# TIERS/multi-modal-loam

Hardware: AMD Instinct MI355X
Metric: scans/s (feature-extract+kNN+10 GN iters) on 16-ring x1800 + Livox 24k fused cloud (higher is better)
Workload: dtype f32/f64; 1 GPU; BASELINE configs[1]: fused VLP-16 16x1800 + Livox Horizon 24000 scan (52800 pts), local map 200000 pts, 1 association pass (thres_dist 25), 10 GN iterations, W=1; resident_slots=8192, stream_lanes=2, distinct_scans=64, map_tiles_touched=43, map_tiles_complete=43, parallelism=scan-sharded x1, device=AMD Radeon Graphics, cus=256

## Files before the change

multi-modal-loam_amd/csrc/lidar_eval.h:

```cpp
#pragma once
#include <math.h>
#include <stddef.h>

#include "mml_internal.h"

namespace {

#ifndef MML_SOLVE_THREADS
#define MML_SOLVE_THREADS 128
#endif
constexpr int SOLVE_THREADS = MML_SOLVE_THREADS;
constexpr int SOLVE_WAVES = SOLVE_THREADS / 64;
constexpr int MAXW = 8;
constexpr double kLidarM = 1.5e-3;

struct Pose {
    double R[9];
    double t[3];
    double tb[3];
    double Jl[9];
};

__device__ void quat_to_R(double qx, double qy, double qz, double qw, double* R) {
    const double tx = 2 * qx, ty = 2 * qy, tz = 2 * qz;
// ... 113 lines not shown
        Pw[0] = __builtin_fma(P.R[2], cz, __builtin_fma(P.R[1], cy, __builtin_fma(P.R[0], cx, P.t[0])));
        Pw[1] = __builtin_fma(P.R[5], cz, __builtin_fma(P.R[4], cy, __builtin_fma(P.R[3], cx, P.t[1])));
        Pw[2] = __builtin_fma(P.R[8], cz, __builtin_fma(P.R[7], cy, __builtin_fma(P.R[6], cx, P.t[2])));
        double l12, il12, a012, ia012, s12, is12, rs, sm14;
        const double dx = ax - bx, dy = ay - by, dz = az - bz;
        sqrt_pair(__builtin_fma(dz, dz, __builtin_fma(dy, dy, dx * dx)), l12, il12);
        const double pax = Pw[0] - ax, pay = Pw[1] - ay, paz = Pw[2] - az, pbx = Pw[0] - bx, pby = Pw[1] - by, pbz = Pw[2] - bz;
        const double c0 = __builtin_fma(pax, pby, -(pbx * pay));
        const double c1 = __builtin_fma(pax, pbz, -(pbx * paz));
        const double c2 = __builtin_fma(pay, pbz, -(pby * paz));
        sqrt_pair(__builtin_fma(c2, c2, __builtin_fma(c1, c1, c0 * c0)), a012, ia012);
        const double ld2 = a012 * il12;
        const double s = __builtin_fma(Pw[2], Pw[2], __builtin_fma(Pw[1], Pw[1], Pw[0] * Pw[0]));
        sqrt_pair(s, s12, is12);
        sqrt_pair(s12, rs, sm14);
        const double weight = 1.0 - 0.9 * fabs(ld2) * sm14;
        const double r = ka * weight * ld2;
        const double ux = c2 * ia012, uy = -c1 * ia012, uz = c0 * ia012;
        double gl[3] = {__builtin_fma(dy, uz, -(dz * uy)) * il12, __builtin_fma(dz, ux, -(dx * uz)) * il12, __builtin_fma(dx, uy, -(dy * ux)) * il12};
        const double sm54 = sm14 * (is12 * is12);
        double gr[3];
        for (int c = 0; c < 3; ++c) {
            double gw = (-0.9) * __builtin_fma(fabs(ld2) * (-0.5) * sm54, Pw[c], sm14 * gl[c]);
            gr[c] = ka * __builtin_fma(ld2, gw, weight * gl[c]);
        }
        double J[6];
        row_jacobian(P, Pw, gr, J);
        double rho0, rho1;
        huber(r * r, huber_delta, rho0, rho1);
        acc[27] += 0.5 * rho0;
        accum(acc, J, r, rho1);
    }
    const double kb = w_tan / kLidarM;
    MmlPlaneFactor nxt;
    if ((int)threadIdx.x < npf) nxt = pf[threadIdx.x];
    for (int i = threadIdx.x; i < npf; i += SOLVE_THREADS) {
        const MmlPlaneFactor f = nxt;
        if (i + SOLVE_THREADS < npf) nxt = pf[i + SOLVE_THREADS];
        if (f.src < 0 || !(fabs(f.error) > 1e-5)) continue;
        const double cx = f.ori[0], cy = f.ori[1], cz = f.ori[2];
        double Pw[3];
        Pw[0] = __builtin_fma(P.R[2], cz, __builtin_fma(P.R[1], cy, __builtin_fma(P.R[0], cx, P.t[0])));
        Pw[1] = __builtin_fma(P.R[5], cz, __builtin_fma(P.R[4], cy, __builtin_fma(P.R[3], cx, P.t[1])));
        Pw[2] = __builtin_fma(P.R[8], cz, __builtin_fma(P.R[7], cy, __builtin_fma(P.R[6], cx, P.t[2])));
        const double d[3] = {Pw[0] - f.proj[0], Pw[1] - f.proj[1], Pw[2] - f.proj[2]};
        double nd, ind, s12, is12, rs, sm14;
        sqrt_pair(__builtin_fma(d[2], d[2], __builtin_fma(d[1], d[1], d[0] * d[0])), nd, ind);
        const double s = __builtin_fma(Pw[2], Pw[2], __builtin_fma(Pw[1], Pw[1], Pw[0] * Pw[0]));
        sqrt_pair(s, s12, is12);
        sqrt_pair(s12, rs, sm14);
        const double weight = 1.0 - 0.9 * nd * sm14;
        const double sm54 = sm14 * (is12 * is12);
        double gw[3];
        const double gwa = sm14 * ind, gwb = nd * (-0.5) * sm54;
        for (int c = 0; c < 3; ++c) gw[c] = (-0.9) * __builtin_fma(gwb, Pw[c], gwa * d[c]);
        const double w[3] = {f.omega[0], f.omega[1], f.omega[2]};
        double rows[3][3];
        int nrows = 1;
        rows[0][0] = ka * w[0];
        rows[0][1] = ka * w[1];
        rows[0][2] = ka * w[2];
        if (kb != 0.0) {
            double h[3] = {0, 0, 0};
            if (fabs(w[0]) <= fabs(w[1]) && fabs(w[0]) <= fabs(w[2]))
                h[0] = 1;
            else if (fabs(w[1]) <= fabs(w[2]))
                h[1] = 1;
            else
                h[2] = 1;
            double t0 = w[1] * h[2] - w[2] * h[1], t1 = w[2] * h[0] - w[0] * h[2], t2 = w[0] * h[1] - w[1] * h[0];
            double n, in;
            sqrt_pair((t0 * t0 + t1 * t1) + t2 * t2, n, in);
            t0 *= in;
            t1 *= in;
            t2 *= in;
            rows[1][0] = kb * t0;
            rows[1][1] = kb * t1;
            rows[1][2] = kb * t2;
            rows[2][0] = kb * (w[1] * t2 - w[2] * t1);
            rows[2][1] = kb * (w[2] * t0 - w[0] * t2);
            rows[2][2] = kb * (w[0] * t1 - w[1] * t0);
            nrows = 3;
        }
        double rr[3], sq = 0;
        for (int q = 0; q < nrows; ++q) {
            rr[q] = weight * __builtin_fma(rows[q][2], d[2], __builtin_fma(rows[q][1], d[1], rows[q][0] * d[0]));
            sq = __builtin_fma(rr[q], rr[q], sq);
        }
        double rho0, rho1;
        huber(sq, huber_delta, rho0, rho1);
        acc[27] += 0.5 * rho0;
        for (int q = 0; q < nrows; ++q) {
            const double rd = __builtin_fma(rows[q][2], d[2], __builtin_fma(rows[q][1], d[1], rows[q][0] * d[0]));
            double gr[3] = {__builtin_fma(rd, gw[0], weight * rows[q][0]), __builtin_fma(rd, gw[1], weight * rows[q][1]),
                            __builtin_fma(rd, gw[2], weight * rows[q][2])};
            double J[6];
            row_jacobian(P, Pw, gr, J);
            accum(acc, J, rr[q], rho1);
        }
    }
}

struct PlaneRow {
    double J[6], rr, rho0, rho1;
    bool valid;
};
__device__ __forceinline__ void plane_row(const MmlPlaneFactor& f, const Pose& P, double ka, double huber_delta, PlaneRow& o) {
    o.valid = !(f.src < 0 || !(fabs(f.error) > 1e-5));
    const double cx = f.ori[0], cy = f.ori[1], cz = f.ori[2];
    double Pw[3];
    Pw[0] = __builtin_fma(P.R[2], cz, __builtin_fma(P.R[1], cy, __builtin_fma(P.R[0], cx, P.t[0])));
    Pw[1] = __builtin_fma(P.R[5], cz, __builtin_fma(P.R[4], cy, __builtin_fma(P.R[3], cx, P.t[1])));
    Pw[2] = __builtin_fma(P.R[8], cz, __builtin_fma(P.R[7], cy, __builtin_fma(P.R[6], cx, P.t[2])));
    const double d[3] = {Pw[0] - f.proj[0], Pw[1] - f.proj[1], Pw[2] - f.proj[2]};
    double nd, ind, s12, is12, rs, sm14;
    sqrt_pair(__builtin_fma(d[2], d[2], __builtin_fma(d[1], d[1], d[0] * d[0])), nd, ind);
    const double s = __builtin_fma(Pw[2], Pw[2], __builtin_fma(Pw[1], Pw[1], Pw[0] * Pw[0]));
    sqrt_pair(s, s12, is12);
    sqrt_pair(s12, rs, sm14);
    const double weight = 1.0 - 0.9 * nd * sm14;
    const double sm54 = sm14 * (is12 * is12);
    double gw[3];
    const double gwa = sm14 * ind, gwb = nd * (-0.5) * sm54;
#pragma unroll
    for (int c = 0; c < 3; ++c) gw[c] = (-0.9) * __builtin_fma(gwb, Pw[c], gwa * d[c]);
    const double row[3] = {ka * (double)f.omega[0], ka * (double)f.omega[1], ka * (double)f.omega[2]};
    o.rr = weight * __builtin_fma(row[2], d[2], __builtin_fma(row[1], d[1], row[0] * d[0]));
    double sq = 0;
    sq = __builtin_fma(o.rr, o.rr, sq);
    huber(sq, huber_delta, o.rho0, o.rho1);
    const double rd = __builtin_fma(row[2], d[2], __builtin_fma(row[1], d[1], row[0] * d[0]));
    double gr[3] = {__builtin_fma(rd, gw[0], weight * row[0]), __builtin_fma(rd, gw[1], weight * row[1]), __builtin_fma(rd, gw[2], weight * row[2])};
    row_jacobian(P, Pw, gr, o.J);
}
__device__ __forceinline__ void eval_frame_pairs(const MmlLineFactor* lf, int nlf, const MmlPlaneFactor* pf, int npf, const Pose& P,
                                 double huber_delta, double* acc) {
    eval_frame(lf, nlf, pf, 0, P, 0.0, huber_delta, acc);
    const double ka = 1.0 / kLidarM;
    for (int i = threadIdx.x; i < npf; i += 2 * SOLVE_THREADS) {
        const bool hb = i + SOLVE_THREADS < npf;
        const MmlPlaneFactor fa = pf[i];
        const MmlPlaneFactor fb = pf[hb ? i + SOLVE_THREADS : i];
        PlaneRow a, b;
        plane_row(fa, P, ka, huber_delta, a);
        plane_row(fb, P, ka, huber_delta, b);
        if (a.valid) {
            acc[27] += 0.5 * a.rho0;
            accum(acc, a.J, a.rr, a.rho1);
        }
        if (hb && b.valid) {
            acc[27] += 0.5 * b.rho0;
            accum(acc, b.J, b.rr, b.rho1);
        }
    }
}

__device__ __forceinline__ double shfl_xor_f64(double v, int o) {
    const unsigned lo = __shfl_xor((unsigned)__double2loint(v), o), hi = __shfl_xor((unsigned)__double2hiint(v), o);
    return __hiloint2double((int)hi, (int)lo);
}
template <int O>
__device__ __forceinline__ unsigned lane_xor_u32(unsigned x, int lane) {
    if constexpr (O == 32) {
        const auto r = __builtin_amdgcn_permlane32_swap(x, x, false, false);
        return lane < 32 ? r[1] : r[0];
    } else if constexpr (O == 16) {
        const auto r = __builtin_amdgcn_permlane16_swap(x, x, false, false);
        return (lane & 16) ? r[0] : r[1];
    } else if constexpr (O == 8) {
        const int m = __builtin_amdgcn_update_dpp(0, (int)x, 0x140, 0xf, 0xf, false);
        return (unsigned)__builtin_amdgcn_update_dpp(0, m, 0x141, 0xf, 0xf, false);
    } else if constexpr (O == 4) {
        const int m = __builtin_amdgcn_update_dpp(0, (int)x, 0x141, 0xf, 0xf, false);
        return (unsigned)__builtin_amdgcn_update_dpp(0, m, 0x1B, 0xf, 0xf, false);
    } else if constexpr (O == 2) {
        return (unsigned)__builtin_amdgcn_update_dpp(0, (int)x, 0x4E, 0xf, 0xf, false);
    } else {
        return (unsigned)__builtin_amdgcn_update_dpp(0, (int)x, 0xB1, 0xf, 0xf, false);
    }
}
template <int O>
__device__ __forceinline__ double lane_xor_f64(double v, int lane) {
    const unsigned lo = lane_xor_u32<O>((unsigned)__double2loint(v), lane), hi = lane_xor_u32<O>((unsigned)__double2hiint(v), lane);
    return __hiloint2double((int)hi, (int)lo);
}

__device__ void block_reduce28(double* acc, double* s_part , double* out) {
    const int lane = threadIdx.x & 63, wave = threadIdx.x >> 6;
    double v[32];
#pragma unroll
    for (int k = 0; k < 32; ++k) v[k] = k < 28 ? acc[k] : 0.0;
    int idx = 0;
#pragma unroll
    for (int c = 16, o = 32; c >= 1; c >>= 1, o >>= 1) {
        const bool up = (lane & o) != 0;
#pragma unroll
        for (int j = 0; j < c; ++j) {
            const double keep = up ? v[j + c] : v[j], send = up ? v[j] : v[j + c];
            v[j] = keep + shfl_xor_f64(send, o);
        }
        idx += up ? c : 0;
    }
    const double tot = v[0] + shfl_xor_f64(v[0], 1);
    if (!(lane & 1) && idx < 28) s_part[wave * 28 + idx] = tot;
    __syncthreads();
    if (threadIdx.x < 28) {
        double r = s_part[threadIdx.x];
        for (int w = 1; w < SOLVE_WAVES; ++w) r += s_part[w * 28 + threadIdx.x];
        out[threadIdx.x] = r;
    }
    __syncthreads();
}

__device__ __forceinline__ void frame_record(const MmlLineFactor* lf, const MmlPlaneFactor* pf, const int* ft_n, int B, int MF, int b,
                                             const double* x6, const double* Tbl, double w_tan, double huber,
                                             double* s_part , double* out) {
    Pose pose;
    make_pose(x6, Tbl, pose);
    double acc[28];
    eval_frame(lf + (size_t)b * MF, ft_n[b], pf + (size_t)b * MF, ft_n[B + b], pose, w_tan, huber, acc);
    block_reduce28(acc, s_part, out);
}

constexpr int WIDE_SUBS = 4;
constexpr int WIDE_THREADS = WIDE_SUBS * SOLVE_THREADS;
constexpr int WIDE_ROUND = 3 * WIDE_SUBS;
constexpr int ROW_DOUBLES = 9;
constexpr int WIDE_ROW_LDS = WIDE_ROUND * ROW_DOUBLES * SOLVE_THREADS;
constexpr int WIDE_SAVE_LDS = 8 * WIDE_THREADS;
static_assert(SOLVE_WAVES == 2, "eval_frame_wide restates block_reduce28 for two wavefronts");

__device__ __forceinline__ void line_row(const MmlLineFactor& f, const Pose& P, double ka, double huber_delta, PlaneRow& o) {
    o.valid = !(f.src < 0 || !(fabs(f.error) > 1e-5));
    const double cx = f.ori[0], cy = f.ori[1], cz = f.ori[2];
    const double ax = f.p1[0], ay = f.p1[1], az = f.p1[2], bx = f.p2[0], by = f.p2[1], bz = f.p2[2];
    double Pw[3];
    Pw[0] = __builtin_fma(P.R[2], cz, __builtin_fma(P.R[1], cy, __builtin_fma(P.R[0], cx, P.t[0])));
    Pw[1] = __builtin_fma(P.R[5], cz, __builtin_fma(P.R[4], cy, __builtin_fma(P.R[3], cx, P.t[1])));
    Pw[2] = __builtin_fma(P.R[8], cz, __builtin_fma(P.R[7], cy, __builtin_fma(P.R[6], cx, P.t[2])));
    double l12, il12, a012, ia012, s12, is12, rs, sm14;
    const double dx = ax - bx, dy = ay - by, dz = az - bz;
    sqrt_pair(__builtin_fma(dz, dz, __builtin_fma(dy, dy, dx * dx)), l12, il12);
    const double pax = Pw[0] - ax, pay = Pw[1] - ay, paz = Pw[2] - az, pbx = Pw[0] - bx, pby = Pw[1] - by, pbz = Pw[2] - bz;
    const double c0 = __builtin_fma(pax, pby, -(pbx * pay));
    const double c1 = __builtin_fma(pax, pbz, -(pbx * paz));
    const double c2 = __builtin_fma(pay, pbz, -(pby * paz));
    sqrt_pair(__builtin_fma(c2, c2, __builtin_fma(c1, c1, c0 * c0)), a012, ia012);
    const double ld2 = a012 * il12;
    const double s = __builtin_fma(Pw[2], Pw[2], __builtin_fma(Pw[1], Pw[1], Pw[0] * Pw[0]));
    sqrt_pair(s, s12, is12);
    sqrt_pair(s12, rs, sm14);
    const double weight = 1.0 - 0.9 * fabs(ld2) * sm14;
    const double r = ka * weight * ld2;
    const double ux = c2 * ia012, uy = -c1 * ia012, uz = c0 * ia012;
    double gl[3] = {__builtin_fma(dy, uz, -(dz * uy)) * il12, __builtin_fma(dz, ux, -(dx * uz)) * il12, __builtin_fma(dx, uy, -(dy * ux)) * il12};
    const double sm54 = sm14 * (is12 * is12);
    double gr[3];
#pragma unroll
    for (int c = 0; c < 3; ++c) {
        double gw = (-0.9) * __builtin_fma(fabs(ld2) * (-0.5) * sm54, Pw[c], sm14 * gl[c]);
        gr[c] = ka * __builtin_fma(ld2, gw, weight * gl[c]);
    }
    row_jacobian(P, Pw, gr, o.J);
    huber(r * r, huber_delta, o.rho0, o.rho1);
    o.rr = r;
}

struct WideRec {
    uint4 q[4];
};
static_assert(sizeof(MmlLineFactor) == 48 && sizeof(MmlPlaneFactor) == 64, "WideRec holds either record");
__device__ __forceinline__ void wide_load(WideRec& r, bool is_line, const MmlLineFactor* lf, int il, const MmlPlaneFactor* pf, int ip) {
    if (is_line) {
        const uint4* p = reinterpret_cast<const uint4*>(lf + il);
        r.q[0] = p[0];
        r.q[1] = p[1];
        r.q[2] = p[2];
    } else {
        const uint4* p = reinterpret_cast<const uint4*>(pf + ip);
        r.q[0] = p[0];
        r.q[1] = p[1];
        r.q[2] = p[2];
        r.q[3] = p[3];
    }
}
__device__ __forceinline__ MmlLineFactor wide_line(const WideRec& r) {
    MmlLineFactor f;
    f.ori[0] = __uint_as_float(r.q[0].x);
    f.ori[1] = __uint_as_float(r.q[0].y);
    f.ori[2] = __uint_as_float(r.q[0].z);
    f.p1[0] = __uint_as_float(r.q[0].w);
    f.p1[1] = __uint_as_float(r.q[1].x);
    f.p1[2] = __uint_as_float(r.q[1].y);
    f.p2[0] = __uint_as_float(r.q[1].z);
    f.p2[1] = __uint_as_float(r.q[1].w);
    f.p2[2] = __uint_as_float(r.q[2].x);
    f.src = (int)r.q[2].y;
    f.error = __hiloint2double((int)r.q[2].w, (int)r.q[2].z);
    return f;
}
__device__ __forceinline__ MmlPlaneFactor wide_plane(const WideRec& r) {
    MmlPlaneFactor f;
    f.ori[0] = __uint_as_float(r.q[0].x);
    f.ori[1] = __uint_as_float(r.q[0].y);
    f.ori[2] = __uint_as_float(r.q[0].z);
    f.omega[0] = __uint_as_float(r.q[0].w);
// ... 230 lines not shown
```

multi-modal-loam_amd/csrc/solve.hip:

```cpp
#include <math.h>
#include <stdlib.h>

#include "lidar_eval.h"
#include "mml_internal.h"
#include "phase_clock.h"

namespace {

__host__ __device__ bool chol6(double* A, double* b) {
    for (int j = 0; j < 6; ++j) {
        double d = A[j * 6 + j];
        for (int k = 0; k < j; ++k) d -= A[j * 6 + k] * A[j * 6 + k];
        if (!(d > 0.0)) return false;
        d = sqrt(d);
        A[j * 6 + j] = d;
        for (int i = j + 1; i < 6; ++i) {
            double s = A[i * 6 + j];
            for (int k = 0; k < j; ++k) s -= A[i * 6 + k] * A[j * 6 + k];
            A[i * 6 + j] = s / d;
        }
    }
    for (int i = 0; i < 6; ++i) {
        double s = b[i];
        for (int k = 0; k < i; ++k) s -= A[i * 6 + k] * b[k];
// ... 897 lines not shown
            }
            return;
        }
        if (fabs(cost - cand) <= 1e-6 * cost) {
            if (lane == 0) {
                S.termination = one + one + one;
                S.go = zero;
            }
            return;
        }
    }
    const double rel = (cost - cand) / S.model_change;
    if (rel > 1e-3) {
        double xc[6], xn = 0, gm = 0;
#pragma unroll
        for (int i = 0; i < 6; ++i) {
            xc[i] = S.xc[i];
            xn += xc[i] * xc[i];
            gm = fmax(gm, fabs(S.recc[21 + i]));
        }
        if (lane < 28) S.rec[lane] = S.recc[lane];
        if (lane == 0) {
#pragma unroll
            for (int i = 0; i < 6; ++i) S.x[i] = xc[i];
            S.x_norm = sqrt(xn);
            S.cost = cand;
            S.successful++;
            if (!fixed && gm <= 1e-10) {
                S.termination = one;
                S.go = zero;
            } else {
                if (rel < 0.25) S.radius *= 0.5;
                if (rel > 0.75) S.radius = fmax(S.radius, 3.0 * S.dogleg_norm);
                S.mu = fmax(1e-8, 2.0 * S.mu / 10.0);
                S.reuse = zero;
            }
        }
    } else if (lane == 0) {
        S.radius *= 0.5;
        S.reuse = one;
    }
}

template <bool SMALL>
__global__ __launch_bounds__(SOLVE_THREADS) void k_solve(SolveParams P) {
    __shared__ TRState S;
    __shared__ double s_part[SOLVE_WAVES * 28];
    __shared__ double s_work[92];
    __shared__ double s_wd[TRW_DOUBLES];
    const int prob = blockIdx.x;
    const int W = P.window;
    const int b0 = P.first + prob * W;
    const int tid = threadIdx.x;
    PhaseClock_sv clk(SV_WATCH(tid == 0 && prob == MML_SV_TIMING));
    clk.count(7);
    if constexpr (SMALL) {
        if (tid < 6 * W) S.x[tid] = S.x_init[tid] = P.x_in ? P.x_in[(size_t)prob * 6 * W + tid] : P.x[(size_t)b0 * 6 + tid];
    } else {
        if (tid < 6 * W) S.x[tid] = S.x_init[tid] = P.x[(size_t)b0 * 6 + tid];
    }
    const bool pairs = SMALL && P.w_tan == 0.0;
    __syncthreads();

    double acc[28];
    for (int f = 0; f < W; ++f) {
        Pose pose;
        make_pose(S.x + 6 * f, P.Tbl, pose);
        const int b = b0 + f;
        if (SMALL && pairs)
            eval_frame_pairs(P.lf + (size_t)b * P.MF, P.ft_n[b], P.pf + (size_t)b * P.MF, P.ft_n[P.B + b], pose, P.huber, acc);
        else
            eval_frame(P.lf + (size_t)b * P.MF, P.ft_n[b], P.pf + (size_t)b * P.MF, P.ft_n[P.B + b], pose, P.w_tan, P.huber, acc);
        block_reduce28(acc, s_part, S.rec + 28 * f);
    }
    if (tid == 0) {
        S.cost = 0;
        double xn = 0;
        for (int f = 0; f < W; ++f) {
            S.cost += S.rec[28 * f + 27];
            for (int i = 0; i < 6; ++i) {
                S.scale[6 * f + i] = 1.0 / (1.0 + sqrt(Hget(S.rec + 28 * f, i, i)));
                xn += S.x[6 * f + i] * S.x[6 * f + i];
            }
        }
        S.x_norm = sqrt(xn);
        S.radius = 1e4;
        S.mu = 1e-8;
        S.reuse = 0;
        S.num_invalid = 0;
        S.iter = 0;
        S.successful = 0;
        S.termination = 0;
        S.go = 1;
        S.alpha = 0;
        S.dogleg_norm = 0;
        P.summ[8 * prob + 2] = S.cost;
        if (!P.fixed) {
            double gm = 0;
            for (int f = 0; f < W; ++f)
                for (int i = 0; i < 6; ++i) gm = fmax(gm, fabs(S.rec[28 * f + 21 + i]));
            if (gm <= 1e-10) {
                S.termination = 1;
                S.go = 0;
            }
        }
    }
    __syncthreads();

    int go = S.go;
    __syncthreads();
    clk.mark(0);
    while (go) {
        if (W == 1) {
            if (tid < 64) tr_propose_w1_wave(S, s_work, P.max_iters);
        } else if (tid == 0) {
            tr_propose(S, W, P.max_iters);
        }
        __syncthreads();
        clk.mark(1);
        go = S.go;
        const int ev = S.evaluate;
        if (!go) break;
        if (ev) {
            for (int f = 0; f < W; ++f) {
                Pose pose;
                make_pose(S.xc + 6 * f, P.Tbl, pose);
                const int b = b0 + f;
                if (SMALL && pairs)
                    eval_frame_pairs(P.lf + (size_t)b * P.MF, P.ft_n[b], P.pf + (size_t)b * P.MF, P.ft_n[P.B + b], pose, P.huber, acc);
                else
                    eval_frame(P.lf + (size_t)b * P.MF, P.ft_n[b], P.pf + (size_t)b * P.MF, P.ft_n[P.B + b], pose, P.w_tan, P.huber, acc);
                clk.mark(2);
                block_reduce28(acc, s_part, S.recc + 28 * f);
                clk.mark(3);
            }
            if (tid < 64) tr_decide_wave(S, s_wd, W, P.fixed);
        }
        __syncthreads();
        clk.mark(4);
        go = S.go;
        if (P.trace && tid < 6 * W) P.trace[((size_t)prob * P.max_iters + (S.iter - 1)) * 6 * W + tid] = S.x[tid];
        __syncthreads();
    }
    if (tid < 6 * W) P.x[(size_t)b0 * 6 + tid] = S.x[tid];
    if (SMALL && P.result && W == 1) {
        double* r = P.result + (size_t)prob * MML_SOLVE_RESULT;
        if (tid < 6) r[tid] = S.x[tid];
        if (tid == 6) r[6] = (double)P.ft_n[b0];
        if (tid == 7) r[7] = (double)P.ft_n[P.B + b0];
        if (tid >= 8 && tid < 24) r[tid] = P.stats ? P.stats[16 * (size_t)b0 + (tid - 8)] : 0.0;
    }
    if (P.trace && tid < 6 * W)
        for (int it = S.iter; it < P.max_iters; ++it) P.trace[((size_t)prob * P.max_iters + it) * 6 * W + tid] = S.x[tid];
    if (tid == 0) {
        double* o = P.summ + 8 * prob;
        o[0] = S.iter;
        o[1] = S.successful;
        o[3] = S.cost;
        o[4] = S.termination;
        o[5] = 0;
    }
}

__global__ __launch_bounds__(WIDE_THREADS) void k_solve_wide(SolveParams P) {
    __shared__ TRState S;
    __shared__ double s_part[SOLVE_WAVES * 28];
    __shared__ double s_work[92];
    __shared__ double s_rows[WIDE_ROW_LDS];
    __shared__ double s_vsave[WIDE_SAVE_LDS];
    static_assert(sizeof(S) + sizeof(s_part) + sizeof(s_work) + sizeof(s_rows) + sizeof(s_vsave) <= 160 * 1024,
                  "k_solve_wide: static LDS beyond gfx950's 160 KiB per workgroup");
    const int prob = blockIdx.x;
    const int b0 = P.first + prob;
    const int tid = threadIdx.x;
    PhaseClock_svw whole(SV_WATCH(tid == 0 && prob == MML_SV_TIMING));
    PhaseClock_sv clk(SV_WATCH(tid == 0 && prob == MML_SV_TIMING));
    if (tid < 6) S.x[tid] = S.x_init[tid] = P.x_in ? P.x_in[(size_t)prob * 6 + tid] : P.x[(size_t)b0 * 6 + tid];
    __syncthreads();
    const MmlLineFactor* lf = P.lf + (size_t)b0 * P.MF;
    const MmlPlaneFactor* pf = P.pf + (size_t)b0 * P.MF;
    const int nlf = P.ft_n[b0], npf = P.ft_n[P.B + b0];
    {
        Pose pose;
        make_pose(S.x, P.Tbl, pose);
        eval_frame_wide(lf, nlf, pf, npf, pose, P.huber, s_rows, s_vsave, s_part, S.rec,
                        PhaseClock_svw(SV_WATCH(tid == 0 && prob == MML_SV_TIMING)));
    }
    if (tid == 0) {
        S.cost = 0;
        double xn = 0;
        S.cost += S.rec[27];
        for (int i = 0; i < 6; ++i) {
            S.scale[i] = 1.0 / (1.0 + sqrt(Hget(S.rec, i, i)));
            xn += S.x[i] * S.x[i];
        }
        S.x_norm = sqrt(xn);
        S.radius = 1e4;
        S.mu = 1e-8;
        S.reuse = 0;
        S.num_invalid = 0;
        S.iter = 0;
        S.successful = 0;
        S.termination = 0;
        S.go = 1;
        S.alpha = 0;
        S.dogleg_norm = 0;
        P.summ[8 * prob + 2] = S.cost;
        if (!P.fixed) {
            double gm = 0;
            for (int i = 0; i < 6; ++i) gm = fmax(gm, fabs(S.rec[21 + i]));
            if (gm <= 1e-10) {
                S.termination = 1;
                S.go = 0;
            }
        }
    }
    __syncthreads();
    int go = S.go;
    __syncthreads();
    while (go) {
        int lane_op = tid;
        asm volatile("" : "+v"(lane_op));
        clk.mark(0);
        if (tid < 64) tr_propose_w1_regs(S, s_work, P.max_iters, lane_op);
        __syncthreads();
        clk.mark(1);
        go = S.go;
        const int ev = S.evaluate;
        if (!go) break;
        if (ev) {
            Pose pose;
            make_pose(S.xc, P.Tbl, pose);
            eval_frame_wide(lf, nlf, pf, npf, pose, P.huber, s_rows, s_vsave, s_part, S.recc,
                            PhaseClock_svw(SV_WATCH(tid == 0 && prob == MML_SV_TIMING)));
            asm volatile("" : "+v"(lane_op));
            clk.mark(0);
            if (tid < 64) tr_decide_w1_regs(S, P.fixed, lane_op);
        }
        __syncthreads();
        clk.mark(4);
        go = S.go;
        if (P.trace && tid < 6) P.trace[((size_t)prob * P.max_iters + (S.iter - 1)) * 6 + tid] = S.x[tid];
        __syncthreads();
    }
    if (tid < 6) P.x[(size_t)b0 * 6 + tid] = S.x[tid];
    if (P.result) {
        double* r = P.result + (size_t)prob * MML_SOLVE_RESULT;
        if (tid < 6) r[tid] = S.x[tid];
        if (tid == 6) r[6] = (double)nlf;
        if (tid == 7) r[7] = (double)npf;
        if (tid >= 8 && tid < 24) r[tid] = P.stats ? P.stats[16 * (size_t)b0 + (tid - 8)] : 0.0;
    }
    if (P.trace && tid < 6)
        for (int it = S.iter; it < P.max_iters; ++it) P.trace[((size_t)prob * P.max_iters + it) * 6 + tid] = S.x[tid];
    if (tid == 0) {
        double* o = P.summ + 8 * prob;
        o[0] = S.iter;
        o[1] = S.successful;
        o[3] = S.cost;
        o[4] = S.termination;
        o[5] = 0;
        whole.mark(5);
        whole.count(6);
    }
}

__global__ __launch_bounds__(SOLVE_THREADS) void k_linearize(int b0, int B, int MF, const int* ft_n,
                                                            const MmlLineFactor* lf, const MmlPlaneFactor* pf,
                                                            const double* x, const double* Tbl, double w_tan,
                                                            double huber_delta, const double* stats, double* record) {
    __shared__ double s_part[SOLVE_WAVES * 28];
    __shared__ double s_out[28];
    const int b = b0 + blockIdx.x;
    x += 6 * blockIdx.x;
    record += 32 * blockIdx.x;
    Pose pose;
    make_pose(x, Tbl, pose);
    double acc[28];
    eval_frame(lf + (size_t)b * MF, ft_n[b], pf + (size_t)b * MF, ft_n[B + b], pose, w_tan, huber_delta, acc);
    block_reduce28(acc, s_part, s_out);
    if (threadIdx.x < 28) record[threadIdx.x] = s_out[threadIdx.x];
    if (threadIdx.x == 0) {
        record[28] = stats[16 * b + 2];
        record[29] = stats[16 * b + 3];
        record[30] = 0;
        record[31] = 0;
    }
}

struct WindowRoundParams {
    int first, n_local, rank, W, B, MF, max_iters, fixed, round, do_eval;
    double huber, w_tan;
    const int* ft_n;
    const MmlLineFactor* lf;
    const MmlPlaneFactor* pf;
    const double* Tbl;
    const double* x_all;
    const double* rec_in;
    double* rec_out;
    TRState* state;
    double* aux;
};

__global__ __launch_bounds__(SOLVE_THREADS) void k_window_round(WindowRoundParams P) {
    __shared__ TRState S;
    __shared__ double s_part[SOLVE_WAVES * 28];
// ... 443 lines not shown
static int launch_solve_frame_parallel(mml_ctx* ctx, int first, int count, int W, const double* d_Tbl, mml_solve_opts opts,
                                       bool second_chunk) {
    if (!ctx->win_state.present()) {
        const int rc = ctx->win_state.reserve(ctx, {MmlPart{&ctx->wstate, sizeof(TRState) * (size_t)ctx->B}, mml_part(ctx->wrec, 2 * 32 * (size_t)ctx->B),
                                                    mml_part(ctx->waux, 4 * (size_t)ctx->B)});
        if (rc != MML_OK) return rc;
    }
    hipStream_t s = MML_STREAM(ctx);
    const int nprob = count / W;
    TRState* st = reinterpret_cast<TRState*>(ctx->wstate) + first;
    double* aux = ctx->waux + 4 * (size_t)first;
    double* rec[2] = {ctx->wrec + 32 * (size_t)first, ctx->wrec + 32 * ((size_t)ctx->B + first)};
    WindowRoundParams P;
    P.first = first;
    P.n_local = 1;
    P.rank = 0;
    P.W = W;
    P.B = ctx->B;
    P.MF = ctx->MF;
    P.max_iters = opts.max_num_iterations;
    P.fixed = opts.fixed_iterations;
    P.huber = opts.huber_delta;
    P.w_tan = opts.plan_weight_tan;
    P.ft_n = ctx->ft_n;
    P.lf = ctx->lf;
    P.pf = ctx->pf;
    P.Tbl = d_Tbl;
    P.x_all = ctx->d_x + 6 * (size_t)first;
    P.state = st;
    P.aux = aux;
    const int rounds = opts.max_num_iterations + 2;
    const int r_begin = second_chunk ? kFirstChunk : 0, r_end = second_chunk ? rounds : (rounds < kFirstChunk ? rounds : kFirstChunk);
    auto enqueue = [&]() -> hipError_t {
        if (!second_chunk) {
            hipError_t e = hipMemsetAsync(st, 0, sizeof(TRState) * (size_t)count, s);
            if (e != hipSuccess) return e;
            e = hipMemsetAsync(aux, 0, sizeof(double) * 4 * (size_t)count, s);
            if (e != hipSuccess) return e;
        }
        for (int r = r_begin; r < r_end; ++r) {
            P.round = r;
            P.do_eval = r + 1 < rounds ? 1 : 0;
            P.rec_in = rec[(r + 1) & 1];
            P.rec_out = rec[r & 1];
            hipLaunchKernelGGL(k_window_round, dim3(W, nprob), dim3(SOLVE_THREADS), 0, s, P);
        }
        hipLaunchKernelGGL(k_window_export, dim3(nprob), dim3(64), 0, s, first, W, st, aux, ctx->d_x, ctx->d_summ + 8 * (size_t)first);
        return hipGetLastError();
    };
    MmlStageScope t(ctx, "solve");
    if (ctx->use_graph) {
        mml_ctx::WinGraph* g = nullptr;
        for (auto& c : ctx->win_graphs)
            if (c.first == first && c.count == count && c.W == W && c.max_iters == opts.max_num_iterations &&
                c.fixed == opts.fixed_iterations && c.huber == opts.huber_delta && c.w_tan == opts.plan_weight_tan && c.stream == s &&
                c.Tbl == d_Tbl && c.second == second_chunk)
                g = &c;
        if (!g && hipStreamBeginCapture(s, hipStreamCaptureModeThreadLocal) == hipSuccess) {
            hipError_t e = enqueue();
            hipGraph_t graph = nullptr;
            hipError_t e2 = hipStreamEndCapture(s, &graph);
            hipGraphExec_t exec = nullptr;
            if (e == hipSuccess && e2 == hipSuccess && graph && hipGraphInstantiate(&exec, graph, nullptr, nullptr, 0) == hipSuccess) {
                if (ctx->win_graphs.size() >= 16) {
                    hipGraphExecDestroy(ctx->win_graphs.front().exec);
                    ctx->win_graphs.erase(ctx->win_graphs.begin());
                }
                mml_ctx::WinGraph c;
                c.first = first;
                c.count = count;
                c.W = W;
                c.max_iters = opts.max_num_iterations;
                c.fixed = opts.fixed_iterations;
                c.huber = opts.huber_delta;
                c.w_tan = opts.plan_weight_tan;
                c.stream = s;
                c.Tbl = d_Tbl;
                c.second = second_chunk;
                c.exec = exec;
                ctx->win_graphs.push_back(c);
                g = &ctx->win_graphs.back();
            }
            if (graph) hipGraphDestroy(graph);
            (void)hipGetLastError();
        }
        if (g) {
            MML_HIP(hipGraphLaunch(g->exec, s));
            return MML_OK;
        }
    }
    MML_HIP(enqueue());
    return MML_OK;
}

int mml_window_solve_continue(mml_ctx* ctx, int first, int count, int window, const double* d_Tbl, mml_solve_opts opts) {
    if (opts.max_num_iterations + 2 <= kFirstChunk) return MML_OK;
    return launch_solve_frame_parallel(ctx, first, count, window, d_Tbl, opts, true);
}

int mml_window_state_read(mml_ctx* ctx, const void* d_state, int W, double* x_window, mml_solve_summary* summ, double initial_cost) {
    TRState* h = new TRState();
    hipError_t e = hipMemcpyAsync(h, d_state, sizeof(TRState), hipMemcpyDeviceToHost, MML_STREAM(ctx));
    if (e == hipSuccess) e = hipStreamSynchronize(MML_STREAM(ctx));
    if (e != hipSuccess) {
        delete h;
        ctx->err = std::string("window state read-back: ") + hipGetErrorString(e);
        return MML_ERR_HIP;
    }
    if (x_window)
        for (int i = 0; i < 6 * W; ++i) x_window[i] = h->x[i];
    if (summ) {
        summ->iterations = h->iter;
        summ->successful = h->successful;
        summ->initial_cost = initial_cost;
        summ->final_cost = h->cost;
        summ->termination = h->termination;
    }
    delete h;
    return MML_OK;
}

int mml_launch_solve(mml_ctx* ctx, int first, int count, int window, const double* d_Tbl, mml_solve_opts opts,
                     bool want_trace, const double* d_x_in, double* d_result) {
    MML_REQUIRE(window >= 1 && window <= MAXW && count % window == 0, MML_ERR_INVALID,
                "window must be in [1,8] and divide count");
    if (window > 1 && !want_trace) return launch_solve_frame_parallel(ctx, first, count, window, d_Tbl, opts, false);
    SolveParams P;
    P.first = first;
    P.B = ctx->B;
    P.MF = ctx->MF;
    P.window = window;
    P.max_iters = opts.max_num_iterations;
    P.fixed = opts.fixed_iterations;
    P.huber = opts.huber_delta;
    P.w_tan = opts.plan_weight_tan;
    P.ft_n = ctx->ft_n;
    P.lf = ctx->lf;
    P.pf = ctx->pf;
    P.Tbl = d_Tbl;
    P.x = ctx->d_x;
    P.summ = ctx->d_summ + 8 * (size_t)first;
    P.trace = want_trace ? ctx->d_trace + (size_t)first * 6 * 64 : nullptr;
    P.x_in = d_x_in;
    P.result = d_result;
    P.stats = ctx->assoc_stats;
    MML_REQUIRE((!d_x_in && !d_result) || window == 1, MML_ERR_INVALID, "packed start poses / result records: one-frame problems only");
    MmlStageScope t(ctx, "solve");
    const bool small = count / window <= ctx->cus;
    MML_REQUIRE((!d_x_in && !d_result) || mml_pose_packed(count, ctx->cus), MML_ERR_INVALID, "packed start poses / result records: packed pose calls only");
    if (small && ctx->solve_wide && window == 1 && opts.plan_weight_tan == 0.0)
        hipLaunchKernelGGL(k_solve_wide, dim3(count), dim3(WIDE_THREADS), 0, MML_STREAM(ctx), P);
    else if (small)
        hipLaunchKernelGGL(k_solve<true>, dim3(count / window), dim3(SOLVE_THREADS), 0, MML_STREAM(ctx), P);
    else
        hipLaunchKernelGGL(k_solve<false>, dim3(count / window), dim3(SOLVE_THREADS), 0, MML_STREAM(ctx), P);
    MML_HIP(hipGetLastError());
    return MML_OK;
}

int mml_launch_linearize(mml_ctx* ctx, int slot, const double* d_x, const double* d_Tbl, double w_tan, double huber,
                         double* d_record, int frames) {
    {
        const int rs = mml_ensure_assoc_stats(ctx, slot, frames);
        if (rs != MML_OK) return rs;
    }
    MmlStageScope t(ctx, "linearize");
    hipLaunchKernelGGL(k_linearize, dim3(frames), dim3(SOLVE_THREADS), 0, MML_STREAM(ctx), slot, ctx->B, ctx->MF, ctx->ft_n,
                       ctx->lf, ctx->pf, d_x, d_Tbl, w_tan, huber, ctx->assoc_stats, d_record);
    MML_HIP(hipGetLastError());
    return MML_OK;
}

struct mml_window_solver {
    TRState S;
    int W;
    mml_solve_opts opts;
    int phase;
    double initial_cost;
};

extern "C" mml_window_solver* mml_window_solver_create(int W, const mml_solve_opts* opts) {
    if (W < 1 || W > MAXW || !opts) return nullptr;
    mml_window_solver* s = new mml_window_solver();
    s->W = W;
    s->opts = *opts;
    s->phase = 0;
    s->initial_cost = 0;
    return s;
}
extern "C" void mml_window_solver_destroy(mml_window_solver* s) { delete s; }

extern "C" int mml_window_solver_step(mml_window_solver* s, const double* records, double* x_eval) {
    if (!s || !records || !x_eval) return MML_ERR_INVALID;
    TRState& S = s->S;
    const int W = s->W, n = 6 * W;
    if (s->phase == 2) {
        for (int i = 0; i < n; ++i) x_eval[i] = S.x[i];
        return 1;
    }
    if (s->phase == 0) {
        for (int f = 0; f < W; ++f) {
            for (int k = 0; k < 28; ++k) S.rec[28 * f + k] = records[MML_NEQ_RECORD_DOUBLES * f + k];
            for (int i = 0; i < 6; ++i) S.x[6 * f + i] = S.x_init[6 * f + i] = x_eval[6 * f + i];
        }
        tr_init(S, W, s->opts.fixed_iterations);
        s->initial_cost = S.cost;
        s->phase = 1;
    } else {
        for (int f = 0; f < W; ++f)
            for (int k = 0; k < 28; ++k) S.recc[28 * f + k] = records[MML_NEQ_RECORD_DOUBLES * f + k];
        tr_decide(S, W, s->opts.fixed_iterations);
    }
    while (S.go) {
        tr_propose(S, W, s->opts.max_num_iterations);
        if (!S.go) break;
        if (S.evaluate) {
            for (int i = 0; i < n; ++i) x_eval[i] = S.xc[i];
            return 0;
        }
    }
    s->phase = 2;
    for (int i = 0; i < n; ++i) x_eval[i] = S.x[i];
    return 1;
}

extern "C" int mml_window_solver_summary(const mml_window_solver* s, mml_solve_summary* out) {
    if (!s || !out) return MML_ERR_INVALID;
    out->iterations = s->S.iter;
    out->successful = s->S.successful;
    out->initial_cost = s->initial_cost;
    out->final_cost = s->S.cost;
    out->termination = s->S.termination;
    return MML_OK;
}
```

Baseline: 450,400 scans/s.

## Add specialized single-frame batch solve kernel with uniform pose and cached first line factor

Adds k_solve_batch1, a dedicated solver kernel for large batches of single-frame problems without tangent weighting or tracing. It builds the pose once in LDS, broadcasts it to scalar registers via readfirstlane, and precomputes each thread's first line factor (including the segment length inverse) once before the GN loop, keeping it in registers across iterations. It also sets waves_per_eu(3) to target higher occupancy and uses a cost-only path in the final fixed iteration. The aim is to cut per-iteration recomputation, register pressure and pose VGPR traffic, at the cost of another kernel variant to maintain and possible register spills.

```diff
diff --git a/multi-modal-loam_amd/csrc/lidar_eval.h b/multi-modal-loam_amd/csrc/lidar_eval.h
--- a/multi-modal-loam_amd/csrc/lidar_eval.h
+++ b/multi-modal-loam_amd/csrc/lidar_eval.h
@@ -289,6 +289,137 @@
             acc[27] += 0.5 * b.rho0;
             accum(acc, b.J, b.rr, b.rho1);
         }
+    }
+}
+
+__device__ __forceinline__ double uniform_f64(double v) {
+    return __hiloint2double(__builtin_amdgcn_readfirstlane(__double2hiint(v)), __builtin_amdgcn_readfirstlane(__double2loint(v)));
+}
+__device__ __forceinline__ void pose_uniform(const Pose& s, Pose& P) {
+#pragma unroll
+    for (int k = 0; k < 9; ++k) {
+        P.R[k] = uniform_f64(s.R[k]);
+        P.Jl[k] = 0.0;
+    }
+#pragma unroll
+    for (int k = 0; k < 3; ++k) {
+        P.t[k] = uniform_f64(s.t[k]);
+        P.tb[k] = 0.0;
+    }
+}
+
+__device__ __forceinline__ Pose pose_at_use(const Pose& P, const Pose* sp) {
+    Pose Q;
+    asm volatile("" ::: "memory");
+#pragma unroll
+    for (int k = 0; k < 9; ++k) Q.Jl[k] = sp->Jl[k];
+#pragma unroll
+    for (int k = 0; k < 3; ++k) Q.tb[k] = sp->tb[k];
+    return Q;
+}
+
+struct LineFixed {
+    float c[3], a[3], b[3];
+    double il12;
+    bool valid;
+};
+__device__ __forceinline__ void line_fixed(const MmlLineFactor& f, LineFixed& o) {
+    o.valid = !(f.src < 0 || !(fabs(f.error) > 1e-5));
+#pragma unroll
+    for (int k = 0; k < 3; ++k) {
+        o.c[k] = f.ori[k];
+        o.a[k] = f.p1[k];
+        o.b[k] = f.p2[k];
+    }
+    const double ax = f.p1[0], ay = f.p1[1], az = f.p1[2], bx = f.p2[0], by = f.p2[1], bz = f.p2[2];
+    double l12;
+    const double dx = ax - bx, dy = ay - by, dz = az - bz;
+    sqrt_pair(__builtin_fma(dz, dz, __builtin_fma(dy, dy, dx * dx)), l12, o.il12);
+}
+__device__ __forceinline__ void line_accum(const LineFixed& L, const Pose& P, const Pose* sp, double ka, double huber_delta, bool cost_only, double* acc) {
+    const double cx = L.c[0], cy = L.c[1], cz = L.c[2];
+    const double ax = L.a[0], ay = L.a[1], az = L.a[2], bx = L.b[0], by = L.b[1], bz = L.b[2];
+    double Pw[3];
+    Pw[0] = __builtin_fma(P.R[2], cz, __builtin_fma(P.R[1], cy, __builtin_fma(P.R[0], cx, P.t[0])));
+    Pw[1] = __builtin_fma(P.R[5], cz, __builtin_fma(P.R[4], cy, __builtin_fma(P.R[3], cx, P.t[1])));
+    Pw[2] = __builtin_fma(P.R[8], cz, __builtin_fma(P.R[7], cy, __builtin_fma(P.R[6], cx, P.t[2])));
+    double a012, ia012, s12, is12, rs, sm14;
+    const double dx = ax - bx, dy = ay - by, dz = az - bz, il12 = L.il12;
+    const double pax = Pw[0] - ax, pay = Pw[1] - ay, paz = Pw[2] - az, pbx = Pw[0] - bx, pby = Pw[1] - by, pbz = Pw[2] - bz;
+    const double c0 = __builtin_fma(pax, pby, -(pbx * pay));
+    const double c1 = __builtin_fma(pax, pbz, -(pbx * paz));
+    const double c2 = __builtin_fma(pay, pbz, -(pby * paz));
+    sqrt_pair(__builtin_fma(c2, c2, __builtin_fma(c1, c1, c0 * c0)), a012, ia012);
+    const double ld2 = a012 * il12;
+    const double s = __builtin_fma(Pw[2], Pw[2], __builtin_fma(Pw[1], Pw[1], Pw[0] * Pw[0]));
+    sqrt_pair(s, s12, is12);
+    sqrt_pair(s12, rs, sm14);
+    const double weight = 1.0 - 0.9 * fabs(ld2) * sm14;
+    const double r = ka * weight * ld2;
+    double rho0, rho1;
+    huber(r * r, huber_delta, rho0, rho1);
+    acc[27] += 0.5 * rho0;
+    if (cost_only) return;
+    const double ux = c2 * ia012, uy = -c1 * ia012, uz = c0 * ia012;
+    double gl[3] = {__builtin_fma(dy, uz, -(dz * uy)) * il12, __builtin_fma(dz, ux, -(dx * uz)) * il12, __builtin_fma(dx, uy, -(dy * ux)) * il12};
+    const double sm54 = sm14 * (is12 * is12);
+    double gr[3];
+#pragma unroll
+    for (int c = 0; c < 3; ++c) {
+        double gw = (-0.9) * __builtin_fma(fabs(ld2) * (-0.5) * sm54, Pw[c], sm14 * gl[c]);
+        gr[c] = ka * __builtin_fma(ld2, gw, weight * gl[c]);
+    }
+    double J[6];
+    row_jacobian(pose_at_use(P, sp), Pw, gr, J);
+    accum(acc, J, r, rho1);
+}
+__device__ __forceinline__ void plane_accum(const MmlPlaneFactor& f, const Pose& P, const Pose* sp, double ka, double huber_delta, bool cost_only, double* acc) {
+    const double cx = f.ori[0], cy = f.ori[1], cz = f.ori[2];
+    double Pw[3];
+    Pw[0] = __builtin_fma(P.R[2], cz, __builtin_fma(P.R[1], cy, __builtin_fma(P.R[0], cx, P.t[0])));
+    Pw[1] = __builtin_fma(P.R[5], cz, __builtin_fma(P.R[4], cy, __builtin_fma(P.R[3], cx, P.t[1])));
+    Pw[2] = __builtin_fma(P.R[8], cz, __builtin_fma(P.R[7], cy, __builtin_fma(P.R[6], cx, P.t[2])));
+    const double d[3] = {Pw[0] - f.proj[0], Pw[1] - f.proj[1], Pw[2] - f.proj[2]};
+    double nd, ind, s12, is12, rs, sm14;
+    sqrt_pair(__builtin_fma(d[2], d[2], __builtin_fma(d[1], d[1], d[0] * d[0])), nd, ind);
+    const double s = __builtin_fma(Pw[2], Pw[2], __builtin_fma(Pw[1], Pw[1], Pw[0] * Pw[0]));
+    sqrt_pair(s, s12, is12);
+    sqrt_pair(s12, rs, sm14);
+    const double weight = 1.0 - 0.9 * nd * sm14;
+    const double row[3] = {ka * (double)f.omega[0], ka * (double)f.omega[1], ka * (double)f.omega[2]};
+    const double rr = weight * __builtin_fma(row[2], d[2], __builtin_fma(row[1], d[1], row[0] * d[0]));
+    double sq = 0;
+    sq = __builtin_fma(rr, rr, sq);
+    double rho0, rho1;
+    huber(sq, huber_delta, rho0, rho1);
+    acc[27] += 0.5 * rho0;
+    if (cost_only) return;
+    const double sm54 = sm14 * (is12 * is12);
+    double gw[3];
+    const double gwa = sm14 * ind, gwb = nd * (-0.5) * sm54;
+#pragma unroll
+    for (int c = 0; c < 3; ++c) gw[c] = (-0.9) * __builtin_fma(gwb, Pw[c], gwa * d[c]);
+    const double rd = __builtin_fma(row[2], d[2], __builtin_fma(row[1], d[1], row[0] * d[0]));
+    double gr[3] = {__builtin_fma(rd, gw[0], weight * row[0]), __builtin_fma(rd, gw[1], weight * row[1]), __builtin_fma(rd, gw[2], weight * row[2])};
+    double J[6];
+    row_jacobian(pose_at_use(P, sp), Pw, gr, J);
+    accum(acc, J, rr, rho1);
+}
+__device__ __forceinline__ void eval_frame_w1(const MmlLineFactor* lf, int nlf, const MmlPlaneFactor* pf, int npf, const Pose& P,
+                                              const Pose* sp, const LineFixed& L0, double huber_delta, bool cost_only, double* acc) {
+#pragma unroll
+    for (int k = 0; k < 28; ++k) acc[k] = 0;
+    const double ka = 1.0 / kLidarM;
+    if (L0.valid) line_accum(L0, P, sp, ka, huber_delta, cost_only, acc);
+    for (int i = threadIdx.x + SOLVE_THREADS; i < nlf; i += SOLVE_THREADS) {
+        LineFixed L;
+        line_fixed(lf[i], L);
+        if (L.valid) line_accum(L, P, sp, ka, huber_delta, cost_only, acc);
+    }
+    for (int i = threadIdx.x; i < npf; i += SOLVE_THREADS) {
+        const MmlPlaneFactor f = pf[i];
+        if (f.src < 0 || !(fabs(f.error) > 1e-5)) continue;
+        plane_accum(f, P, sp, ka, huber_delta, cost_only, acc);
     }
 }
 
diff --git a/multi-modal-loam_amd/csrc/solve.hip b/multi-modal-loam_amd/csrc/solve.hip
--- a/multi-modal-loam_amd/csrc/solve.hip
+++ b/multi-modal-loam_amd/csrc/solve.hip
@@ -1073,6 +1073,121 @@
     }
     if (P.trace && tid < 6 * W)
         for (int it = S.iter; it < P.max_iters; ++it) P.trace[((size_t)prob * P.max_iters + it) * 6 * W + tid] = S.x[tid];
+    if (tid == 0) {
+        double* o = P.summ + 8 * prob;
+        o[0] = S.iter;
+        o[1] = S.successful;
+        o[3] = S.cost;
+        o[4] = S.termination;
+        o[5] = 0;
+    }
+}
+
+__global__ __launch_bounds__(SOLVE_THREADS) __attribute__((amdgpu_waves_per_eu(3))) void k_solve_batch1(SolveParams P) {
+    __shared__ TRState S;
+    __shared__ double s_part[SOLVE_WAVES * 28];
+    __shared__ double s_work[92];
+    __shared__ double s_wd[TRW_DOUBLES];
+    __shared__ Pose s_pose;
+    static_assert(3 * 2 * (sizeof(TRState) + sizeof(s_part) + sizeof(s_work) + sizeof(s_wd) + sizeof(Pose)) <= 160 * 1024,
+                  "k_solve_batch1: three wavefronts per SIMD are six workgroups per CU");
+    const int prob = blockIdx.x;
+    const int b0 = P.first + prob;
+    const int tid = threadIdx.x;
+    PhaseClock_sv clk(SV_WATCH(tid == 0 && prob == MML_SV_TIMING));
+    clk.count(7);
+    const MmlLineFactor* lf = P.lf + (size_t)b0 * P.MF;
+    const MmlPlaneFactor* pf = P.pf + (size_t)b0 * P.MF;
+    const int nlf = max(P.ft_n[b0], 0), npf = max(P.ft_n[P.B + b0], 0);
+    if (tid < 6) S.x[tid] = S.x_init[tid] = P.x[(size_t)b0 * 6 + tid];
+    if (tid < 64) {
+        __builtin_amdgcn_wave_barrier();
+        asm volatile("" ::: "memory");
+        Pose pose;
+        make_pose(S.x, P.Tbl, pose);
+        if (tid == 0) s_pose = pose;
+    }
+    LineFixed L0;
+    L0.valid = false;
+    if (tid < nlf) line_fixed(lf[tid], L0);
+    __syncthreads();
+
+    double acc[28];
+    {
+        Pose pose;
+        pose_uniform(s_pose, pose);
+        eval_frame_w1(lf, nlf, pf, npf, pose, &s_pose, L0, P.huber, false, acc);
+        block_reduce28(acc, s_part, S.rec);
+    }
+    if (tid == 0) {
+        S.cost = 0;
+        double xn = 0;
+        S.cost += S.rec[27];
+        for (int i = 0; i < 6; ++i) {
+            S.scale[i] = 1.0 / (1.0 + sqrt(Hget(S.rec, i, i)));
+            xn += S.x[i] * S.x[i];
+        }
+        S.x_norm = sqrt(xn);
+        S.radius = 1e4;
+        S.mu = 1e-8;
+        S.reuse = 0;
+        S.num_invalid = 0;
+        S.iter = 0;
+        S.successful = 0;
+        S.termination = 0;
+        S.go = 1;
+        S.alpha = 0;
+        S.dogleg_norm = 0;
+        P.summ[8 * prob + 2] = S.cost;
+        if (!P.fixed) {
+            double gm = 0;
+            for (int i = 0; i < 6; ++i) gm = fmax(gm, fabs(S.rec[21 + i]));
+            if (gm <= 1e-10) {
+                S.termination = 1;
+                S.go = 0;
+            }
+        }
+    }
+    __syncthreads();
+
+    int go = S.go;
+    __syncthreads();
+    clk.mark(0);
+    while (go) {
+        int lane_op = tid;
+        asm volatile("" : "+v"(lane_op));
+        if (tid < 64) {
+            tr_propose_w1_wave(S, s_work, P.max_iters, lane_op);
+            __builtin_amdgcn_wave_barrier();
+            asm volatile("" ::: "memory");
+            if (S.go && S.evaluate) {
+                Pose pose;
+                make_pose(S.xc, P.Tbl, pose);
+                if (tid == 0) s_pose = pose;
+            }
+        }
+        __syncthreads();
+        clk.mark(1);
+        go = S.go;
+        const int ev = S.evaluate;
+        if (!go) break;
+        if (ev) {
+            const bool cost_only = P.fixed && S.iter >= P.max_iters;
+            Pose pose;
+            pose_uniform(s_pose, pose);
+            eval_frame_w1(lf, nlf, pf, npf, pose, &s_pose, L0, P.huber, cost_only, acc);
+            clk.mark(2);
+            block_reduce28(acc, s_part, S.recc);
+            clk.mark(3);
+            asm volatile("" : "+v"(lane_op));
+            if (tid < 64) tr_decide_wave(S, s_wd, 1, P.fixed, lane_op);
+        }
+        __syncthreads();
+        clk.mark(4);
+        go = S.go;
+        __syncthreads();
+    }
+    if (tid < 6) P.x[(size_t)b0 * 6 + tid] = S.x[tid];
     if (tid == 0) {
         double* o = P.summ + 8 * prob;
         o[0] = S.iter;
@@ -1822,6 +1937,8 @@
         hipLaunchKernelGGL(k_solve_wide, dim3(count), dim3(WIDE_THREADS), 0, MML_STREAM(ctx), P);
     else if (small)
         hipLaunchKernelGGL(k_solve<true>, dim3(count / window), dim3(SOLVE_THREADS), 0, MML_STREAM(ctx), P);
+    else if (window == 1 && opts.plan_weight_tan == 0.0 && !want_trace)
+        hipLaunchKernelGGL(k_solve_batch1, dim3(count), dim3(SOLVE_THREADS), 0, MML_STREAM(ctx), P);
     else
         hipLaunchKernelGGL(k_solve<false>, dim3(count / window), dim3(SOLVE_THREADS), 0, MML_STREAM(ctx), P);
     MML_HIP(hipGetLastError());
```

New measurement: 456,900 scans/s, median of 6. 1.4% higher.
